# bluenote-1577/sylph

Measured on AMD Instinct MI355X. Metric: read Gbp/s sketched + genome-comparisons/s profiled, 1 Gbp vs GTDB-R220, higher is better.
Workload: dtype u64

## Files before the change

sylph_amd/csrc/common.h:

```cpp
#pragma once
#include <hip/hip_runtime.h>

#include <atomic>
#include <cstdarg>
#include <cstdint>
#include <cstdio>
#include <cstdlib>
#include <cstring>
#include <ctime>
#include <map>
#include <mutex>
#include <string>
#include <vector>

#include "../../include/sylph_hip.h"

struct sylph_ctx;

namespace sylph {

void set_error(const char* fmt, ...);

struct HipError { hipError_t e; const char* what; const char* file; int line; };

// ... 49 lines not shown

void* pool_acquire(sylph_ctx* ctx, size_t bytes, size_t* cap_out);
void pool_release(sylph_ctx* ctx, void* p, size_t cap);

struct DevBuf {
    void* p = nullptr;
    size_t cap = 0;
    sylph_ctx* ctx = nullptr;
    DevBuf() = default;
    explicit DevBuf(sylph_ctx* c) : ctx(c) {}
    DevBuf(const DevBuf&) = delete;
    DevBuf& operator=(const DevBuf&) = delete;
    ~DevBuf() { release(); }
    void release() {
        if (p) {
            if (ctx) pool_release(ctx, p, cap);
            else (void)hipFree(p);
        }
        p = nullptr;
        cap = 0;
    }
    void alloc(size_t want) {
        if (ctx) p = pool_acquire(ctx, want, &cap);
        else { SY_HIP(hipMalloc(&p, want)); cap = want; }
    }
    void reserve(size_t bytes) {
        if (bytes <= cap) return;
        release();
        alloc(bytes + bytes / 4 + 256);
    }
    void grow_keep(size_t bytes, size_t keep, hipStream_t s) {
        if (bytes <= cap) return;
        void* old = p;
        const size_t old_cap = cap;
        p = nullptr;
        cap = 0;
        alloc(bytes * 2 + 256);
        if (keep && old) SY_HIP(hipMemcpyAsync(p, old, keep, hipMemcpyDeviceToDevice, s));
        if (old) {
            if (ctx) pool_release(ctx, old, old_cap);
            else { SY_HIP(hipStreamSynchronize(s)); (void)hipFree(old); }
        }
    }
    template <class T> T* as() const { return reinterpret_cast<T*>(p); }
};

struct KernelStat { double ms = 0; uint64_t launches = 0; };

}

#ifndef SYLPH_READS_TAIL_PCT
#define SYLPH_READS_TAIL_PCT 10
#endif
struct sylph_ctx {
    int device = 0;
    hipStream_t stream = nullptr;
    bool own_stream = false;
    std::mutex mu;
    int finish_mode = 0;
    uint32_t bucket_target = 128;
    uint32_t plain_records = 1;
    uint32_t shard_reduce = 0;
    uint32_t fail_next_peer_copy = 0;
    uint32_t fail_next_shard_probe = 0;
    uint32_t index_lambda = 0;
    uint64_t index_pass_max = 1ull << 30;
    struct SeedTurn { hipEvent_t gate = nullptr, done = nullptr; bool recorded = false; } turn;
    void seed_gate() { if (turn.gate) { (void)hipStreamWaitEvent(stream, turn.gate, 0); turn.gate = nullptr; } }
    void seed_done() { if (turn.done && !turn.recorded && hipEventRecord(turn.done, stream) == hipSuccess) turn.recorded = true; }
    std::string profile_only;
    uint32_t reads_tail_pct = SYLPH_READS_TAIL_PCT;
    int reads_hash = -1;
    uint32_t reads_slack = 0;
    uint32_t reads_wg_per_cu = 0;
    uint64_t push_chunk_bytes = 64ull << 20;
    int seeds_mode = 0;
    std::atomic<int> refs{1};
    bool profile = false;
    std::map<std::string, sylph::KernelStat> stats;
    struct Pending { std::string fam; hipEvent_t a, b; };
    std::vector<Pending> pending;
    std::vector<hipEvent_t> event_pool;
    std::vector<std::pair<size_t, void*>> pool_free;
    size_t pool_bytes = 0;
    sylph::DevBuf tmp_sort;
    sylph::DevBuf scratch[8];
    sylph::DevBuf counters;
    void* pinned = nullptr;
    void read_back(void* dst, const void* dev_src, size_t bytes);
    static constexpr size_t STAGE_BYTES = 32u << 20;
    void* stage[2] = {nullptr, nullptr};
    hipEvent_t stage_ev[2] = {nullptr, nullptr};
    hipStream_t copy_stream = nullptr;
    hipEvent_t copy_ev[2] = {nullptr, nullptr};
    void d2h(void* dst, const void* dev_src, size_t bytes);
    void h2d(void* dev_dst, const void* src, size_t bytes);
};

namespace sylph {

struct ScopedKernelTimer {
    sylph_ctx* ctx;
    hipEvent_t a = nullptr, b = nullptr;
    const char* fam;
    ScopedKernelTimer(sylph_ctx* c, const char* family);
    ~ScopedKernelTimer();
};
void profile_collect(sylph_ctx* ctx);
void ctx_unref(sylph_ctx* ctx);

struct HostPhase {
    sylph_ctx* ctx;
    const char* name;
// ... 36 lines not shown
```

sylph_amd/csrc/partition.h:

```cpp
#pragma once
#include "common.h"
#include "device_common.h"
#include "sketch_session.h"

namespace sylph {
namespace {

struct BucketMap { int sh; uint32_t mult; uint32_t B; int composite; uint32_t range_hs; uint32_t sub_mult[3]; uint32_t sub_width[3]; int rank_bits[3]; };

__device__ __forceinline__ uint32_t bucket_of_key(uint32_t key, const BucketMap m) { return min(__umulhi(key, m.mult), m.B - 1u); }
__device__ __forceinline__ uint64_t bucket_lo_hash(uint32_t b, uint32_t mult, int sh) { return ((((uint64_t)b << 32) + mult - 1u) / mult) << sh; }
__device__ __forceinline__ uint32_t sub_range_of(uint32_t res, uint32_t sub_mult, uint32_t cap) {
    return sub_mult ? min(__umulhi(res, sub_mult), cap - 1u) : min(res, cap - 1u);
}
__device__ __forceinline__ uint32_t take_place(uint16_t* fill, uint32_t bin) {
    const uint32_t old = atomicAdd(reinterpret_cast<uint32_t*>(fill) + (bin >> 1), (bin & 1u) ? 65536u : 1u);
    return (bin & 1u) ? (old >> 16) : (old & 0xFFFFu);
}

struct PartIn {
    const uint64_t* hash;
    const uint32_t* slot_key;
    const uint32_t* blk_count;
    uint32_t n_dense, n_blk, slot_cap, tile_entries;
    uint32_t blk_per_tile;
    int slotted, key_sh;
    uint32_t stage_pairs;
    int carry;
};
constexpr int PART_TPB = 256;
constexpr uint32_t BLK_PER_TILE = 16;
constexpr uint32_t MAX_COARSE = 4096;
constexpr uint32_t MAX_FINE = 4096;
#ifndef SYLPH_STAGE_PAIRS
#define SYLPH_STAGE_PAIRS 4096
#endif
constexpr uint32_t STAGE_PAIRS = SYLPH_STAGE_PAIRS;

__device__ __forceinline__ uint32_t xcd_tile(uint32_t n_tiles) {
    const uint32_t per_xcd = (n_tiles + 7) / 8;
    return (blockIdx.x & 7u) * per_xcd + (blockIdx.x >> 3);
}

template <class F>
__device__ __forceinline__ void for_tile_entries(const PartIn& in, uint32_t t, F&& f) {
    if (in.slotted == 1) {
        const uint32_t grp = threadIdx.x >> 5, l = threadIdx.x & 31;
        for (uint32_t bl = grp; bl < in.blk_per_tile; bl += PART_TPB / 32) {
            const uint32_t b = t * in.blk_per_tile + bl;
            if (b >= in.n_blk) break;
            const uint32_t cnt = min(in.blk_count[b], in.slot_cap), g0 = b * in.slot_cap;
            for (uint32_t i = l; i < cnt; i += 32) f(in.slot_key[g0 + i], g0 + i, 0ull);
        }
    } else if (in.slotted == 2) {
        const uint32_t grp = threadIdx.x >> 5, l = threadIdx.x & 31;
        for (uint32_t bl = grp; bl < in.blk_per_tile; bl += PART_TPB / 32) {
            const uint32_t b = t * in.blk_per_tile + bl;
            if (b >= in.n_blk) break;
            const uint32_t cnt = 2u * min(in.blk_count[b], in.slot_cap), g0 = 2u * b * in.slot_cap;
            for (uint32_t i = l; i < cnt; i += 32) {
                const uint64_t h = in.hash[g0 + i];
                if (h != INVALID_HASH) f((uint32_t)(h >> in.key_sh), g0 + i, h);
            }
        }
// ... 250 lines not shown
```

sylph_amd/csrc/replay_lds.hip:

```cpp
#include "common.h"
#include "device_common.h"
#include "sketch_session.h"
#include "partition.h"

namespace sylph {
namespace {

#ifndef SYLPH_REPLAY_TPB
#define SYLPH_REPLAY_TPB 128
#endif
constexpr int CAP_SMALL = 256, RTPB_SMALL = SYLPH_REPLAY_TPB;
constexpr int CAP_MID = 512, RTPB_MID = 256;
constexpr int CAP_LARGE = 1024, RTPB_LARGE = 256;
constexpr int IDX_BITS = 10;
constexpr uint32_t SEG_LIMIT = 96;


struct ReplayArgs {
    const OccRec* recs;
    const uint64_t* hash;
    const uint32_t* perm;
    const uint32_t* boff;
    const uint32_t* p_nv;
    int paired, dedup;
    uint32_t cutoff;
    BucketMap bm;
    uint64_t* tmp_k;
    uint32_t* tmp_c;
    uint32_t* n_distinct;
    uint32_t* removed_b;
    uint32_t* overflow;
    uint32_t* mid_list;
    uint32_t* large_list;
    uint32_t* ovf_list;
    int dbg_stage;
};

struct FinishTail {
    unsigned long long removed;
    uint32_t overflow;
    uint32_t n_seg;
    uint32_t n_ovf, n_mid, n_large;
    uint32_t verdict[2];
    uint32_t a10_words[2];
    uint32_t n_found;
};
static_assert(sizeof(FinishTail) == 48, "tail block");

__device__ __forceinline__ uint32_t marker_tag(uint64_t m) { return (uint32_t)((m * 0x9E3779B97F4A7C15ull) >> 49) | 1u; }

template <int CAP, int RTPB>
__device__ __forceinline__ void replay_bucket(const uint32_t b, const ReplayArgs& ra) {
    const OccRec* __restrict__ recs = ra.recs;
    const uint32_t* __restrict__ perm = ra.perm;
    const uint32_t* __restrict__ boff = ra.boff;
    uint64_t* __restrict__ tmp_k = ra.tmp_k;
    uint32_t* __restrict__ tmp_c = ra.tmp_c;
    uint32_t* __restrict__ n_distinct = ra.n_distinct;
    uint32_t* __restrict__ mid_list = ra.mid_list;
    const int paired = ra.paired, dbg_stage = ra.dbg_stage;
    const uint32_t cutoff = ra.cutoff;
    const BucketMap& bm = ra.bm;
    constexpr int ITEMS = CAP / RTPB;
    const bool filter = ra.dedup == DEDUP_FILTER;
    const int no_dedup = filter ? 0 : ra.dedup;
    __shared__ uint64_t s_hash[CAP], s_rid[CAP], s_m0[CAP], s_m1[CAP];
    __shared__ __attribute__((aligned(8))) uint16_t s_seg[CAP];
    __shared__ uint8_t s_fl[CAP];
    __shared__ __attribute__((aligned(8))) uint16_t s_ab[2 * (CAP + 2)];
    uint16_t* const s_a = s_ab;
    uint16_t* const s_b = s_ab + (CAP + 2);
    __shared__ uint32_t s_wave[RTPB / 64];
    const uint32_t tid = threadIdx.x;
    const uint32_t nv = *ra.p_nv;
    const uint32_t first = boff[b], last = boff[b + 1];
    const uint32_t n = last - first;
    if (last > nv || first > last) { if (tid == 0) atomicAdd(ra.overflow, 1u); return; }
    if (n == 0) return;
    if (n > CAP) {
        if (tid == 0) {
            uint32_t* list = (CAP < CAP_MID && n <= (uint32_t)CAP_MID) ? mid_list : (CAP < CAP_LARGE && n <= (uint32_t)CAP_LARGE) ? ra.large_list : ra.ovf_list;
            list[1 + atomicAdd(&list[0], 1u)] = b;
        }
        return;
    }
    uint64_t* s_key = s_m0;
    const bool composite = bm.composite != 0;
    const uint64_t lo_hash = composite ? bucket_lo_hash(b, bm.mult, bm.sh) : 0ull;
    OccRec r[ITEMS];
    uint32_t pidx[ITEMS], rank[ITEMS];
    constexpr bool SEG_DIRECT = CAP == CAP_SMALL;
    uint32_t seg0[ITEMS];
#pragma unroll
    for (int q = 0; q < ITEMS; q++) seg0[q] = 0;
    uint32_t* const s_pidx = reinterpret_cast<uint32_t*>(s_rid);
    const int levels = (int)((n + RTPB - 1) / RTPB);
#pragma unroll
    for (int q = 0; q < ITEMS; q++) pidx[q] = perm[first + min(tid + q * RTPB, n - 1u)];
#pragma unroll
    for (int q = 0; q < ITEMS; q++) r[q] = recs[pidx[q]];
#pragma unroll
    for (int q = 0; q < ITEMS; q++) {
        rank[q] = 0;
        if (tid + q * RTPB >= n) pidx[q] = 0xFFFFFFFFu;
    }
    if (composite) {
        uint32_t* const s_cnt = reinterpret_cast<uint32_t*>(s_m1);
        const uint32_t sub_mult = bm.sub_mult[CAP == CAP_SMALL ? 0 : CAP == CAP_MID ? 1 : 2];
        uint32_t sub[ITEMS];
        constexpr int CFG = CAP == CAP_SMALL ? 0 : CAP == CAP_MID ? 1 : 2;
        const int rank_bits = bm.rank_bits[CFG];
        constexpr bool TWO_LEVEL = CAP != CAP_SMALL;
        unsigned long long* const s_min = reinterpret_cast<unsigned long long*>(s_hash);
        unsigned long long* const s_max = reinterpret_cast<unsigned long long*>(s_rid);
        for (uint32_t t = tid; t <= (uint32_t)CAP; t += RTPB) s_cnt[t] = 0;
        for (uint32_t t = tid; t < (uint32_t)CAP / 2; t += RTPB) reinterpret_cast<uint32_t*>(s_seg)[t] = 0;
        if constexpr (TWO_LEVEL)
            for (uint32_t t = tid; t < (uint32_t)CAP; t += RTPB) { s_min[t] = ~0ull; s_max[t] = 0ull; }
        __syncthreads();
#pragma unroll
        for (int q = 0; q < ITEMS; q++) {
            const uint32_t i = tid + q * RTPB;
            sub[q] = 0;
            if (i < n) {
                sub[q] = sub_range_of((uint32_t)((r[q].hash - lo_hash) >> bm.sh), sub_mult, CAP);
// ... 376 lines not shown
    {
        uint32_t rc = base_c;
        for (uint32_t t = 0; t < items; t++) {
            const uint32_t j = j0 + t;
            if (j >= n) break;
            s_b[j] = (uint16_t)rc;
            if (cbits & (1u << t)) rc++;
        }
        if (j0 < n && j0 + items >= n) s_b[n] = (uint16_t)rc;
    }
    __syncthreads();
    }
    if constexpr (HASHED) {
        uint16_t* const s_headpos = s_a;
        {
            uint32_t rh = base_h;
            for (uint32_t t = 0; t < items; t++) {
                const uint32_t j = j0 + t;
                if (j >= n) break;
                if (headbits & (1u << t)) s_headpos[rh++] = (uint16_t)j;
            }
            if (tid == 0) s_headpos[total_heads] = (uint16_t)n;
        }
        __syncthreads();
        uint32_t rh = base_h;
        for (uint32_t t = 0; t < items; t++) {
            const uint32_t j = j0 + t;
            if (j >= n) break;
            if (headbits & (1u << t)) {
                const uint32_t e = s_headpos[rh + 1];
                tmp_k[first + rh] = s_hash[j];
                tmp_c[first + rh] = (uint32_t)s_b[e] - (uint32_t)s_b[j];
                rh++;
            }
        }
    } else {
        uint32_t rh = base_h;
        const uint32_t out0 = first;
        for (uint32_t t = 0; t < items; t++) {
            const uint32_t j = j0 + t;
            if (j >= n) break;
            if (headbits & (1u << t)) {
                uint32_t e = j + 1;
                while (e < n && s_seg[e] == j) e++;
                tmp_k[out0 + rh] = s_hash[j];
                tmp_c[out0 + rh] = (uint32_t)s_b[e] - (uint32_t)s_b[j];
                rh++;
            }
        }
    }
    if (tid == 0) { n_distinct[b] = total_heads; ra.removed_b[b] = total_removed; }
}

template <int CAP, int RTPB>
__global__ __launch_bounds__(RTPB) void bucket_replay_kernel(ReplayArgs ra) {
    replay_bucket<CAP, RTPB>(blockIdx.x, ra);
}

template <int CAP, int RTPB>
__device__ __forceinline__ void count_bucket(const uint32_t b, const ReplayArgs& ra) {
    const uint64_t* __restrict__ hash = ra.hash;
    const uint32_t* __restrict__ perm = ra.perm;
    const uint32_t* __restrict__ boff = ra.boff;
    uint64_t* __restrict__ tmp_k = ra.tmp_k;
    uint32_t* __restrict__ tmp_c = ra.tmp_c;
    const BucketMap& bm = ra.bm;
    constexpr int ITEMS = CAP / RTPB;
    __shared__ uint64_t s_key[CAP], s_sorted[CAP];
    __shared__ uint32_t s_cnt[CAP + 1], s_mult[CAP];
    __shared__ __attribute__((aligned(8))) uint16_t s_fill[CAP];
    __shared__ uint32_t s_wave[RTPB / 64];
    const uint32_t tid = threadIdx.x;
    const uint32_t nv = *ra.p_nv;
    const uint32_t first = boff[b], last = boff[b + 1];
    const uint32_t n = last - first;
    if (last > nv || first > last) { if (tid == 0) atomicAdd(ra.overflow, 1u); return; }
    if (n == 0) return;
    if (n > (uint32_t)CAP) {
        if (tid == 0) {
            uint32_t* list = (CAP < CAP_LARGE && n <= (uint32_t)CAP_LARGE) ? ra.large_list : ra.ovf_list;
            list[1 + atomicAdd(&list[0], 1u)] = b;
        }
        return;
    }
    const uint64_t lo_hash = bucket_lo_hash(b, bm.mult, bm.sh);
    const uint32_t sub_mult = bm.sub_mult[CAP == CAP_SMALL ? 0 : CAP == CAP_MID ? 1 : 2];
    uint64_t h[ITEMS];
    uint32_t sub[ITEMS], place[ITEMS];
#pragma unroll
    for (int q = 0; q < ITEMS; q++) {
        const uint32_t i = tid + q * RTPB;
        h[q] = i < n ? (perm ? hash[perm[first + i]] : hash[first + i]) : 0ull;
    }
    for (uint32_t t = tid; t <= (uint32_t)CAP; t += RTPB) s_cnt[t] = 0;
    for (uint32_t t = tid; t < (uint32_t)CAP; t += RTPB) s_fill[t] = 0;
    __syncthreads();
#pragma unroll
    for (int q = 0; q < ITEMS; q++) {
        const uint32_t i = tid + q * RTPB;
        sub[q] = 0;
        if (i < n) {
            sub[q] = sub_range_of((uint32_t)((h[q] - lo_hash) >> bm.sh), sub_mult, CAP);
            atomicAdd(&s_cnt[sub[q]], 1u);
        }
    }
    __syncthreads();
    scan_counters<CAP, RTPB>(s_cnt, s_cnt, s_wave);
    __syncthreads();
#pragma unroll
// ... 7 lines not shown
    }
    __syncthreads();
#pragma unroll
    for (int q = 0; q < ITEMS; q++) {
        const uint32_t i = tid + q * RTPB;
        if (i < n) {
            const uint32_t lo = s_cnt[sub[q]], hi = s_cnt[sub[q] + 1];
            uint32_t less = 0, eq = 0, eq_before = 0;
            for (uint32_t p = lo; p < hi; p++) {
                const uint64_t kp = s_key[p];
                less += kp < h[q] ? 1u : 0u;
                const uint32_t same = kp == h[q] ? 1u : 0u;
                eq += same;
                eq_before += (same && p < place[q]) ? 1u : 0u;
            }
            const uint32_t r = lo + less + eq_before;
            s_sorted[r] = h[q];
            s_mult[r] = eq_before == 0 ? eq : 0u;
        }
    }
    __syncthreads();
    const uint32_t items = (n + RTPB - 1) / RTPB, j0 = tid * items;
    uint32_t heads = 0;
    for (uint32_t t = 0; t < items; t++) {
        const uint32_t j = j0 + t;
        if (j >= n) break;
        heads += s_mult[j] ? 1u : 0u;
    }
    uint32_t total_heads = 0;
    uint32_t rh = block_excl_sum<RTPB>(heads, s_wave, &total_heads);
    for (uint32_t t = 0; t < items; t++) {
        const uint32_t j = j0 + t;
        if (j >= n) break;
        const uint32_t m = s_mult[j];
        if (m) { tmp_k[first + rh] = s_sorted[j]; tmp_c[first + rh] = m; rh++; }
    }
    if (tid == 0) { ra.n_distinct[b] = total_heads; ra.removed_b[b] = 0; }
}
template <int CAP, int RTPB>
__global__ __launch_bounds__(RTPB) void bucket_count_kernel(ReplayArgs ra) {
    count_bucket<CAP, RTPB>(blockIdx.x, ra);
}
template <int CAP, int RTPB>
__global__ __launch_bounds__(RTPB) void bucket_count_list_kernel(ReplayArgs ra, const uint32_t* __restrict__ my_list) {
    const uint32_t n_listed = my_list[0];
    for (uint32_t i = blockIdx.x; i < n_listed; i += gridDim.x) {
        count_bucket<CAP, RTPB>(my_list[1 + i], ra);
        __syncthreads();
    }
}
template <int CAP, int RTPB>
__global__ __launch_bounds__(RTPB) void bucket_replay_list_kernel(ReplayArgs ra, const uint32_t* __restrict__ my_list) {
    const uint32_t n_listed = my_list[0];
    for (uint32_t i = blockIdx.x; i < n_listed; i += gridDim.x) {
        replay_bucket<CAP, RTPB>(my_list[1 + i], ra);
        __syncthreads();
    }
}

constexpr uint32_t SCAN_CHUNK = 1024;
__global__ __launch_bounds__(SCAN_CHUNK) void table_scan_kernel(const uint32_t* __restrict__ n_distinct, const uint32_t* __restrict__ removed_b,
                                                                uint32_t B, uint32_t ipt, uint32_t* __restrict__ d_loc,
                                                                uint32_t* __restrict__ chunk_rows, unsigned long long* __restrict__ chunk_removed) {
    __shared__ uint32_t s_wave[SCAN_CHUNK / 64];
    __shared__ unsigned long long s_rem[SCAN_CHUNK / 64];
    const uint32_t b0 = (blockIdx.x * SCAN_CHUNK + threadIdx.x) * ipt, lane = threadIdx.x & 63, wave = threadIdx.x >> 6;
    uint32_t v = 0;
    unsigned long long rem = 0;
    for (uint32_t i = 0; i < ipt && b0 + i < B; i++) { v += n_distinct[b0 + i]; rem += removed_b[b0 + i]; }
    uint32_t x = v;
#pragma unroll
    for (int d = 1; d < 64; d <<= 1) {
        const uint32_t y = __shfl_up(x, d);
        if (lane >= (uint32_t)d) x += y;
    }
#pragma unroll
    for (int d = 32; d > 0; d >>= 1) rem += __shfl_xor(rem, d);
    if (lane == 63) s_wave[wave] = x;
    if (lane == 0) s_rem[wave] = rem;
    __syncthreads();
    uint32_t base = 0, tot = 0;
    for (uint32_t w = 0; w < SCAN_CHUNK / 64; w++) { const uint32_t t = s_wave[w]; if (w < wave) base += t; tot += t; }
    uint32_t run = base + x - v;
    for (uint32_t i = 0; i < ipt && b0 + i < B; i++) { d_loc[b0 + i] = run; run += n_distinct[b0 + i]; }
    if (threadIdx.x == 0) {
        unsigned long long r = 0;
        for (uint32_t w = 0; w < SCAN_CHUNK / 64; w++) r += s_rem[w];
        chunk_rows[blockIdx.x] = tot;
        chunk_removed[blockIdx.x] = r;
    }
}
__global__ __launch_bounds__(256) void table_compact_kernel(const uint64_t* __restrict__ tmp_k, const uint32_t* __restrict__ tmp_c,
                                                            const uint32_t* __restrict__ boff, const uint32_t* __restrict__ d_loc,
                                                            const uint32_t* __restrict__ chunk_rows, const unsigned long long* __restrict__ chunk_removed,
                                                            const uint32_t* __restrict__ n_distinct, uint32_t B, uint32_t ipt,
                                                            uint64_t* __restrict__ out_k, uint32_t* __restrict__ out_c,
                                                            const uint32_t* __restrict__ ovf_list, const uint32_t* __restrict__ mid_list,
                                                            const uint32_t* __restrict__ large_list, int skip_if_listed,
                                                            FinishTail* __restrict__ tail, const uint32_t* __restrict__ verdict,
                                                            const uint32_t* __restrict__ a10_words, const uint32_t* __restrict__ p_nv) {
    __shared__ uint32_t s_base[257];
    __shared__ uint32_t s_wave[4];
    __shared__ unsigned long long s_rem[4];
    const uint32_t chunk = SCAN_CHUNK * ipt, n_chunks = (B + chunk - 1) / chunk;
    {
        const uint32_t v = threadIdx.x < n_chunks ? chunk_rows[threadIdx.x] : 0u;
        uint32_t tot = 0;
        const uint32_t ex = block_excl_sum<256>(v, s_wave, &tot);
// ... 35 lines not shown
        uint32_t run = 0;
        for (uint32_t t = 0; t < 1024; t++) { const uint32_t v = s_part[t]; s_part[t] = run; run += v; }
        sub_off[m] = run;
    }
    __syncthreads();
    uint32_t run = s_part[tid];
    for (uint32_t i = tid * per; i < min(m, (tid + 1) * per); i++) {
        const uint32_t b = ovf_list[1 + i];
        sub_off[i] = run;
        run += boff[b + 1] - boff[b];
    }
}

__global__ __launch_bounds__(256) void ovf_indices_kernel(const uint32_t* __restrict__ ovf_list, const uint32_t* __restrict__ sub_off,
                                                          const uint32_t* __restrict__ boff, const uint32_t* __restrict__ perm,
                                                          uint32_t* __restrict__ sub_idx) {
    const uint32_t b = ovf_list[1 + blockIdx.x], first = boff[b], n = boff[b + 1] - first, o = sub_off[blockIdx.x];
    for (uint32_t j = threadIdx.x; j < n; j += blockDim.x) sub_idx[o + j] = perm[first + j];
}
__global__ __launch_bounds__(256) void ovf_gather_kernel(const uint32_t* __restrict__ sorted_idx, uint32_t n, const OccRec* __restrict__ recs,
                                                         uint64_t* __restrict__ sub_hash, OccRec* __restrict__ sub_recs) {
    const uint32_t j = blockIdx.x * blockDim.x + threadIdx.x;
    if (j >= n) return;
    const OccRec r = recs[sorted_idx[j]];
    sub_hash[j] = r.hash;
    sub_recs[j] = r;
}

__global__ __launch_bounds__(256) void ovf_patch_kernel(const uint32_t* __restrict__ ovf_list, BucketMap bm,
                                                        const uint64_t* __restrict__ sub_k, const uint32_t* __restrict__ sub_c,
                                                        uint32_t n_sub_out, const uint32_t* __restrict__ boff,
                                                        uint64_t* __restrict__ tmp_k, uint32_t* __restrict__ tmp_c,
                                                        uint32_t* __restrict__ n_distinct) {
    const uint32_t b = ovf_list[1 + blockIdx.x];
    auto lower = [&](uint64_t key) {
        uint32_t lo = 0, hi = n_sub_out;
        while (lo < hi) {
            const uint32_t mid = lo + ((hi - lo) >> 1);
            if (sub_k[mid] < key) lo = mid + 1; else hi = mid;
        }
        return lo;
    };
    __shared__ uint32_t s_lo, s_hi;
    if (threadIdx.x == 0) {
        s_lo = lower(bucket_lo_hash(b, bm.mult, bm.sh));
        s_hi = (b + 1 < bm.B) ? lower(bucket_lo_hash(b + 1, bm.mult, bm.sh)) : n_sub_out;
    }
    __syncthreads();
    const uint32_t lo = s_lo, n = s_hi - s_lo, d = boff[b];
    for (uint32_t i = threadIdx.x; i < n; i += blockDim.x) { tmp_k[d + i] = sub_k[lo + i]; tmp_c[d + i] = sub_c[lo + i]; }
    if (threadIdx.x == 0) n_distinct[b] = n;
}

uint32_t grid_of(uint64_t n, uint32_t tpb = 256) { return (uint32_t)((n + tpb - 1) / tpb); }

}

bool finish_bucketed(sylph_sketch* sk) {
    sylph_ctx* ctx = sk->ctx;
    const bool slotted = sk->pend.live;
    const bool deferred = slotted && sk->pend.deferred;
    const uint32_t n_cap = slotted ? sk->pend.n : (uint32_t)sk->n_occ;
    const uint32_t n_all = deferred ? std::max<uint32_t>(1, sk->pend.n_expect) : n_cap;
    sk->n_out = 0;
    sk->dup_removed = 0;
    if (n_cap == 0) return true;
    if (sk->c < 2) return false;
    const uint64_t thr = UINT64_MAX / (uint64_t)sk->c;
    const uint32_t TARGET = ctx->bucket_target;
    const uint32_t B = (uint32_t)std::min<uint64_t>(std::max<uint64_t>(1, n_all / TARGET), 1u << 24);
    BucketMap bm;
    bm.sh = key_shift(sk->c);
    const uint64_t hs_max = thr >> bm.sh;
    bm.mult = (uint32_t)std::min<uint64_t>(0xFFFFFFFFull, ((uint64_t)B << 32) / (hs_max + 1));
    bm.B = B;
    const uint64_t range_hs = (0x100000000ull + bm.mult - 1) / std::max<uint32_t>(1, bm.mult) + 1;
    bm.composite = bm.mult >= 1 && bit_length(range_hs) + bm.sh <= 64 - IDX_BITS;
    bm.range_hs = (uint32_t)std::min<uint64_t>(range_hs, 0xFFFFFFFFull);
    {
        const uint32_t caps[3] = {(uint32_t)CAP_SMALL, (uint32_t)CAP_MID, (uint32_t)CAP_LARGE};
        for (int i = 0; i < 3; i++) bm.sub_mult[i] = range_hs > caps[i] ? (uint32_t)(((uint64_t)caps[i] << 32) / range_hs) : 0u;
        const uint64_t max_index = slotted ? (uint64_t)sk->pend.n_blk * sk->pend.slot_cap : (uint64_t)n_all;
        const int index_bits = bit_length(max_index | 1);
        for (int i = 0; i < 3; i++) {
            bm.sub_width[i] = bm.sub_mult[i] ? (uint32_t)(range_hs / caps[i]) : 1u;
            uint64_t span_hs = 1;
            if (bm.sub_mult[i]) {
                const uint64_t top = std::min<uint64_t>(range_hs, (((uint64_t)caps[i] << 32) + bm.sub_mult[i] - 1) / bm.sub_mult[i]);
                span_hs = top - (uint64_t)(caps[i] - 1) * bm.sub_width[i] + 1;
            }
            bm.rank_bits[i] = (bm.composite && bit_length(span_hs) + bm.sh + index_bits <= 64) ? index_bits : 0;
        }
    }
    const PartGeom geom = part_geometry(B);
    if (!slotted && sk->n_plain && !(sk->n_plain == sk->n_occ && bm.composite)) materialise_plain_records(sk);
    bool plain = !slotted && sk->n_plain != 0;
    static const uint32_t tile_blocks = [] { const char* e = getenv("SYLPH_HIP_PART_TILE_BLOCKS"); return e ? (uint32_t)std::max(1, std::min(32, atoi(e))) : BLK_PER_TILE; }();
    static const uint32_t stage_pairs = [] { const char* e = getenv("SYLPH_HIP_PART_STAGE_PAIRS"); return e ? (uint32_t)std::max(256, std::min(8192, atoi(e))) : 2048u; }();
    PartIn in{};
    in.slotted = slotted ? 1 : 0;
    in.key_sh = bm.sh;
    uint32_t n_tiles;
    const OccRec* recs;
    if (slotted) {
        in.slot_key = sk->slot_key.as<uint32_t>();
        in.n_blk = sk->pend.n_blk;
        in.slot_cap = sk->pend.slot_cap;
        in.blk_count = sk->slot_meta.as<uint32_t>() + (sk->pend.n_blk + 1);
        in.blk_per_tile = tile_blocks;
        in.stage_pairs = stage_pairs;
        n_tiles = (in.n_blk + tile_blocks - 1) / tile_blocks;
        recs = sk->slot_rec.as<OccRec>();
    } else {
        in.hash = sk->hash.as<uint64_t>();
        in.n_dense = n_all;
        in.tile_entries = (uint32_t)std::max<uint64_t>(4096, ((uint64_t)n_all + 65535) / 65536);
        n_tiles = (uint32_t)(((uint64_t)n_all + in.tile_entries - 1) / in.tile_entries);
        recs = sk->recs.as<OccRec>();
    }
    DevBuf &b_hist = ctx->scratch[0], &b_pairs = ctx->scratch[1], &b_perm = ctx->scratch[2], &b_tmpk = ctx->scratch[3],
           &b_tmpc = ctx->scratch[4], &b_small = ctx->scratch[5], &b_bk = ctx->scratch[6];
    b_hist.reserve(part_hist_words(geom, n_tiles) * 4);
    b_pairs.reserve((size_t)n_cap * 8);
    if (!plain) b_perm.reserve((size_t)n_cap * 4);
    DevBuf& b_sorted = ctx->scratch[7];
    if (plain) b_sorted.reserve((size_t)n_cap * 8);
    uint64_t* sorted_hash = plain ? b_sorted.as<uint64_t>() : nullptr;
    in.carry = plain ? 1 : 0;
    b_tmpk.reserve((size_t)n_cap * 8);
    b_tmpc.reserve((size_t)n_cap * 4);
    b_small.reserve(64);
    b_bk.reserve((size_t)(B + 2) * 4 * 7 + 264 * 4 + 264 * 8 + 16);
    uint32_t* hist = b_hist.as<uint32_t>();
    uint2* pairs = b_pairs.as<uint2>();
    uint32_t* boff = b_bk.as<uint32_t>();
    uint32_t* large_list = boff + (B + 2);
    uint32_t* ovf_list = large_list + (B + 2);
    uint32_t* n_distinct = ovf_list + (B + 2);
    uint32_t* removed_b = n_distinct + (B + 2);
    uint32_t* d_off = removed_b + (B + 2);
    uint32_t* mid_list = d_off + (B + 2);
    uint32_t* chunk_rows = mid_list + (B + 2) + ((B & 1u) ? 1 : 0);
    unsigned long long* chunk_removed = reinterpret_cast<unsigned long long*>(chunk_rows + 264);
    FinishTail* d_tail = b_small.as<FinishTail>();
    const uint32_t* d_nv = boff + B;
    const uint32_t n_zero = (B + 2) * 2;
    const int dbg = getenv("SYLPH_REPLAY_STAGE") ? atoi(getenv("SYLPH_REPLAY_STAGE")) : 0;
    const uint32_t cutoff = sk->paired ? 0u : 4u;
    sk->out_k.reserve((size_t)n_cap * 8);
    sk->out_c.reserve((size_t)n_cap * 4);
    ReplayArgs ra{};
    if (plain) ra.hash = sorted_hash;
    else { ra.recs = recs; ra.perm = b_perm.as<uint32_t>(); }
    ra.boff = boff; ra.p_nv = d_nv;
    ra.paired = sk->paired; ra.dedup = sk->dedup_mode(); ra.cutoff = cutoff; ra.bm = bm;
    ra.tmp_k = b_tmpk.as<uint64_t>(); ra.tmp_c = b_tmpc.as<uint32_t>(); ra.n_distinct = n_distinct; ra.removed_b = removed_b;
    ra.overflow = &d_tail->overflow;
    ra.mid_list = mid_list; ra.large_list = large_list; ra.ovf_list = ovf_list; ra.dbg_stage = dbg;
    {
        HostPhase ph(ctx, "finish(bucket): partition + LDS replay + compact");
        {
            ScopedKernelTimer t(ctx, "sort");
            launch_partition(ctx, in, bm, geom, n_tiles, n_all, hist, pairs, boff, b_perm.as<uint32_t>(), sorted_hash, n_distinct, n_zero,
                             b_small.as<uint32_t>(), large_list, ovf_list, mid_list);
        }
        {
            ScopedKernelTimer t(ctx, "replay");
            if (plain) hipLaunchKernelGGL((bucket_count_kernel<CAP_SMALL, RTPB_SMALL>), dim3(B), dim3(RTPB_SMALL), 0, ctx->stream, ra);
            else hipLaunchKernelGGL((bucket_replay_kernel<CAP_SMALL, RTPB_SMALL>), dim3(B), dim3(RTPB_SMALL), 0, ctx->stream, ra);
        }
    }
    auto close_table = [&](int skip_if_listed) {
        const uint32_t ipt = (B + (1u << 18) - 1) >> 18;
        ScopedKernelTimer t(ctx, "replay");
        hipLaunchKernelGGL(table_scan_kernel, dim3((B + SCAN_CHUNK * ipt - 1) / (SCAN_CHUNK * ipt)), dim3(SCAN_CHUNK), 0, ctx->stream, n_distinct,
                           removed_b, B, ipt, d_off, chunk_rows, chunk_removed);
        hipLaunchKernelGGL(table_compact_kernel, dim3(std::min<uint32_t>((B + 3) / 4, 1u << 15)), dim3(256), 0, ctx->stream,
                           b_tmpk.as<uint64_t>(), b_tmpc.as<uint32_t>(), boff, d_off, chunk_rows, chunk_removed, n_distinct, B, ipt,
                           sk->out_k.as<uint64_t>(), sk->out_c.as<uint32_t>(), ovf_list, mid_list, large_list, skip_if_listed,
                           d_tail, deferred ? sk->slot_meta.as<uint32_t>() + (size_t)(sk->pend.n_blk + 1) * 4 : (const uint32_t*)nullptr,
                           sk->a10_state == 1 ? sk->a10_tail.as<uint32_t>() : (const uint32_t*)nullptr, d_nv);
        SY_HIP(hipGetLastError());
    };
    FinishTail host{};
    auto read_tail = [&] {
        SY_HIP(hipMemcpyAsync(ctx->pinned, d_tail, sizeof host, hipMemcpyDeviceToHost, ctx->stream));
        SY_HIP(hipStreamSynchronize(ctx->stream));
        memcpy(&host, ctx->pinned, sizeof host);
        if (!ctx->pending.empty()) profile_collect(ctx);
    };
    close_table(1);
    read_tail();
    if (deferred) {
        if (host.verdict[0] || host.verdict[1]) {
            redo_deferred_batch(sk);
            a10_mark(sk);
            return finish_bucketed(sk);
        }
        sk->pend.deferred = false;
        sk->pend.n = host.n_found;
    }
    if (!a10_verdict(sk, host.a10_words)) return finish_bucketed(sk);
    if (host.overflow) return false;
    if (plain && host.n_ovf) {
        materialise_plain_records(sk);
        return finish_bucketed(sk);
    }
    if (host.n_mid || host.n_large) {
        HostPhase ph(ctx, "finish(bucket): medium / large configurations");
        {
            ScopedKernelTimer t(ctx, "replay");
            if (plain) {
                if (host.n_large)
                    hipLaunchKernelGGL((bucket_count_list_kernel<CAP_LARGE, RTPB_LARGE>), dim3(std::min<uint32_t>(host.n_large, 1536u)),
                                       dim3(RTPB_LARGE), 0, ctx->stream, ra, large_list);
            } else {
                if (host.n_mid)
                    hipLaunchKernelGGL((bucket_replay_list_kernel<CAP_MID, RTPB_MID>), dim3(std::min<uint32_t>(host.n_mid, 1280u)),
                                       dim3(RTPB_MID), 0, ctx->stream, ra, mid_list);
                if (host.n_large)
                    hipLaunchKernelGGL((bucket_replay_list_kernel<CAP_LARGE, RTPB_LARGE>), dim3(std::min<uint32_t>(host.n_large, 512u)),
                                       dim3(RTPB_LARGE), 0, ctx->stream, ra, large_list);
            }
        }
        close_table(0);
        read_tail();
        if (host.overflow) return false;
    }
    unsigned long long removed_extra = 0;
    if (host.n_ovf) {
        if (ctx->finish_mode == 2 || host.n_ovf > 4096) return false;
        HostPhase ph(ctx, "finish(bucket): overflowing buckets through the device-wide path");
        const uint32_t m = host.n_ovf;
        DevBuf b_so(ctx), b_si(ctx), b_sh(ctx), b_sr(ctx), sub_k(ctx), sub_c(ctx);
        b_so.reserve(((size_t)m + 1) * 4);
        hipLaunchKernelGGL(ovf_offsets_kernel, dim3(1), dim3(1024), 0, ctx->stream, ovf_list, boff, b_so.as<uint32_t>());
        uint32_t n_sub = 0;
        ctx->read_back(&n_sub, b_so.as<uint32_t>() + m, 4);
        b_si.reserve((size_t)n_sub * 8);
        b_sh.reserve((size_t)n_sub * 8);
        b_sr.reserve((size_t)n_sub * sizeof(OccRec));
        uint32_t* sub_idx = b_si.as<uint32_t>();
        uint32_t* sub_sorted = sub_idx + n_sub;
        hipLaunchKernelGGL(ovf_indices_kernel, dim3(m), dim3(256), 0, ctx->stream, ovf_list, b_so.as<uint32_t>(), boff,
                           b_perm.as<uint32_t>(), sub_idx);
        sort_keys_u32(ctx, sub_idx, sub_sorted, n_sub, 0, 32);
        {
            ScopedKernelTimer t(ctx, "replay_overflow");
            hipLaunchKernelGGL(ovf_gather_kernel, dim3(grid_of(n_sub)), dim3(256), 0, ctx->stream, sub_sorted, n_sub, recs,
                               b_sh.as<uint64_t>(), b_sr.as<OccRec>());
        }
        uint64_t n_sub_out = 0, removed_sub = 0;
        generic_replay(ctx, b_sh.as<uint64_t>(), b_sr.as<OccRec>(), n_sub, sk->paired, sk->dedup_mode(), sub_k, sub_c, n_sub_out, removed_sub);
        removed_extra = removed_sub;
        {
            ScopedKernelTimer t(ctx, "replay");
// ... 13 lines not shown
```

Before: 1110.

## Add a single-pass lane path for small buckets in replay and lower bucket target

Adds a specialized replay body for buckets holding at most 128 records. Each thread owns one record, ranks it by a direct count within its sub-range, and deduplicates without the general multi-item sort machinery. Specialised instances are templated on paired/dedup mode. The default bucket target drops from 128 to 96 so more buckets fit the lane path. The change also adds a reciprocal-based bucket low-key computation, moves shared memory into a struct shared by both bodies, and adds profiling counters; the extra template instances and the SGPR cap may raise register pressure.

New measurement: 1134, median of 6. +2.2%, better.

```diff
diff --git a/sylph_amd/csrc/common.h b/sylph_amd/csrc/common.h
--- a/sylph_amd/csrc/common.h
+++ b/sylph_amd/csrc/common.h
@@ -125,13 +125,16 @@
 #ifndef SYLPH_READS_TAIL_PCT
 #define SYLPH_READS_TAIL_PCT 10
 #endif
+#ifndef SYLPH_BUCKET_TARGET
+#define SYLPH_BUCKET_TARGET 96
+#endif
 struct sylph_ctx {
     int device = 0;
     hipStream_t stream = nullptr;
     bool own_stream = false;
     std::mutex mu;
     int finish_mode = 0;
-    uint32_t bucket_target = 128;
+    uint32_t bucket_target = SYLPH_BUCKET_TARGET;
     uint32_t plain_records = 1;
     uint32_t shard_reduce = 0;
     uint32_t fail_next_peer_copy = 0;
diff --git a/sylph_amd/csrc/partition.h b/sylph_amd/csrc/partition.h
--- a/sylph_amd/csrc/partition.h
+++ b/sylph_amd/csrc/partition.h
@@ -6,10 +6,16 @@
 namespace sylph {
 namespace {
 
-struct BucketMap { int sh; uint32_t mult; uint32_t B; int composite; uint32_t range_hs; uint32_t sub_mult[3]; uint32_t sub_width[3]; int rank_bits[3]; };
+struct BucketMap { int sh; uint32_t mult; uint32_t B; int composite; uint32_t range_hs; uint32_t sub_mult[4]; uint32_t sub_width[4]; int rank_bits[4]; uint64_t inv_mult; };
 
 __device__ __forceinline__ uint32_t bucket_of_key(uint32_t key, const BucketMap m) { return min(__umulhi(key, m.mult), m.B - 1u); }
 __device__ __forceinline__ uint64_t bucket_lo_hash(uint32_t b, uint32_t mult, int sh) { return ((((uint64_t)b << 32) + mult - 1u) / mult) << sh; }
+__device__ __forceinline__ uint64_t bucket_lo_key(uint32_t b, uint32_t mult, uint64_t inv) {
+    uint64_t q = (uint64_t)b * (uint32_t)(inv >> 32) + (((uint64_t)b * (uint32_t)inv) >> 32);
+    uint64_t r = ((uint64_t)b << 32) - q * mult;
+    if (r >= mult) { q++; r -= mult; }
+    return q + (r ? 1u : 0u);
+}
 __device__ __forceinline__ uint32_t sub_range_of(uint32_t res, uint32_t sub_mult, uint32_t cap) {
     return sub_mult ? min(__umulhi(res, sub_mult), cap - 1u) : min(res, cap - 1u);
 }
diff --git a/sylph_amd/csrc/replay_lds.hip b/sylph_amd/csrc/replay_lds.hip
--- a/sylph_amd/csrc/replay_lds.hip
+++ b/sylph_amd/csrc/replay_lds.hip
@@ -14,6 +14,8 @@
 constexpr int CAP_LARGE = 1024, RTPB_LARGE = 256;
 constexpr int IDX_BITS = 10;
 constexpr uint32_t SEG_LIMIT = 96;
+constexpr uint32_t SINGLE_CUTOFF = 4;
+constexpr int LANE_CAP = 128, LANE_CFG = 3;
 
 
 struct ReplayArgs {
@@ -47,10 +49,19 @@
 };
 static_assert(sizeof(FinishTail) == 48, "tail block");
 
+template <int CAP, int RTPB>
+struct ReplayLds {
+    uint64_t hash[CAP], rid[CAP], m0[CAP], m1[CAP];
+    __attribute__((aligned(8))) uint16_t seg[CAP];
+    uint8_t fl[CAP];
+    __attribute__((aligned(8))) uint16_t ab[2 * (CAP + 2)];
+    uint32_t wave[RTPB / 64];
+};
+
 __device__ __forceinline__ uint32_t marker_tag(uint64_t m) { return (uint32_t)((m * 0x9E3779B97F4A7C15ull) >> 49) | 1u; }
 
 template <int CAP, int RTPB>
-__device__ __forceinline__ void replay_bucket(const uint32_t b, const ReplayArgs& ra) {
+__device__ __forceinline__ void replay_bucket(const uint32_t b, const ReplayArgs& ra, ReplayLds<CAP, RTPB>& lds) {
     const OccRec* __restrict__ recs = ra.recs;
     const uint32_t* __restrict__ perm = ra.perm;
     const uint32_t* __restrict__ boff = ra.boff;
@@ -64,13 +75,13 @@
     constexpr int ITEMS = CAP / RTPB;
     const bool filter = ra.dedup == DEDUP_FILTER;
     const int no_dedup = filter ? 0 : ra.dedup;
-    __shared__ uint64_t s_hash[CAP], s_rid[CAP], s_m0[CAP], s_m1[CAP];
-    __shared__ __attribute__((aligned(8))) uint16_t s_seg[CAP];
-    __shared__ uint8_t s_fl[CAP];
-    __shared__ __attribute__((aligned(8))) uint16_t s_ab[2 * (CAP + 2)];
+    uint64_t* const s_hash = lds.hash, * const s_rid = lds.rid, * const s_m0 = lds.m0, * const s_m1 = lds.m1;
+    uint16_t* const s_seg = lds.seg;
+    uint8_t* const s_fl = lds.fl;
+    uint16_t* const s_ab = lds.ab;
     uint16_t* const s_a = s_ab;
     uint16_t* const s_b = s_ab + (CAP + 2);
-    __shared__ uint32_t s_wave[RTPB / 64];
+    uint32_t* const s_wave = lds.wave;
     const uint32_t tid = threadIdx.x;
     const uint32_t nv = *ra.p_nv;
     const uint32_t first = boff[b], last = boff[b + 1];
@@ -553,9 +564,181 @@
     if (tid == 0) { n_distinct[b] = total_heads; ra.removed_b[b] = total_removed; }
 }
 
-template <int CAP, int RTPB>
-__global__ __launch_bounds__(RTPB) void bucket_replay_kernel(ReplayArgs ra) {
-    replay_bucket<CAP, RTPB>(blockIdx.x, ra);
+template <bool PAIRED, int DEDUP>
+__device__ __forceinline__ void replay_bucket_lane(const uint32_t b, const uint32_t first, const uint32_t n, const ReplayArgs& ra,
+                                                   ReplayLds<CAP_SMALL, LANE_CAP>& lds) {
+    const OccRec* __restrict__ recs = ra.recs;
+    const uint32_t* __restrict__ perm = ra.perm;
+    uint64_t* __restrict__ tmp_k = ra.tmp_k;
+    uint32_t* __restrict__ tmp_c = ra.tmp_c;
+    const BucketMap& bm = ra.bm;
+    constexpr bool filter = DEDUP == DEDUP_FILTER, no_dedup = DEDUP == DEDUP_NONE;
+    uint64_t* const s_hash = lds.hash, * const s_rid = lds.rid, * const s_m0 = lds.m0, * const s_m1 = lds.m1;
+    uint16_t* const s_seg = lds.seg;
+    uint16_t* const s_a = lds.ab;
+    uint16_t* const s_b = lds.ab + (CAP_SMALL + 2);
+    uint32_t* const s_wave = lds.wave;
+    const uint32_t tid = threadIdx.x;
+    const bool live = tid < n;
+    const uint32_t pidx = perm[first + min(tid, n - 1u)];
+    const OccRec r = recs[pidx];
+    const uint64_t lo_hash = bucket_lo_key(b, bm.mult, bm.inv_mult) << bm.sh;
+    const int rank_bits = bm.rank_bits[LANE_CFG];
+    uint64_t* const s_key = s_m0;
+    uint32_t* const s_cnt = reinterpret_cast<uint32_t*>(s_m1);
+    uint16_t* const s_fill = s_seg;
+    s_cnt[tid] = 0;
+    if (tid == 0) s_cnt[LANE_CAP] = 0;
+    if (tid < LANE_CAP / 2) reinterpret_cast<uint32_t*>(s_seg)[tid] = 0;
+    __syncthreads();
+    uint32_t sub = 0;
+    if (live) {
+        sub = sub_range_of((uint32_t)((r.hash - lo_hash) >> bm.sh), bm.sub_mult[LANE_CFG], LANE_CAP);
+        atomicAdd(&s_cnt[sub], 1u);
+    }
+    __syncthreads();
+    {
+        const bool deep = scan_counters<LANE_CAP, LANE_CAP>(s_cnt, s_cnt, s_wave) >= SEG_LIMIT;
+        if constexpr (!no_dedup) {
+            if (__syncthreads_or(deep)) {
+                if (tid == 0) ra.mid_list[1 + atomicAdd(&ra.mid_list[0], 1u)] = b;
+                return;
+            }
+        } else
+            __syncthreads();
+    }
+    uint64_t rkey = 0;
+    if (live) {
+        const uint32_t place = s_cnt[sub] + take_place(s_fill, sub);
+        const uint64_t res = (r.hash - lo_hash) - ((uint64_t)(sub * bm.sub_width[LANE_CFG]) << bm.sh);
+        rkey = (res << rank_bits) | pidx;
+        s_key[place] = rkey;
+    }
+    __syncthreads();
+    uint32_t rank = 0, seg0 = 0;
+    if (live) {
+        const uint32_t lo = s_cnt[sub], hi = s_cnt[sub + 1];
+        const uint64_t hkey = rkey & ~((1ull << rank_bits) - 1ull);
+        uint32_t smaller = 0, below = 0;
+        for (uint32_t p = lo; p < hi; p++) {
+            const uint64_t kp = s_key[p];
+            smaller += kp < rkey ? 1u : 0u;
+            below += kp < hkey ? 1u : 0u;
+        }
+        rank = lo + smaller;
+        seg0 = lo + below;
+    }
+    __syncthreads();
+    if (live) {
+        s_hash[rank] = r.hash; s_rid[rank] = r.rid; s_m0[rank] = r.m0; s_m1[rank] = r.m1;
+        s_seg[rank] = (uint16_t)seg0;
+    }
+    __syncthreads();
+    const uint32_t j = tid;
+    const uint32_t seg = live ? (uint32_t)s_seg[j] : 0u;
+    const bool head = live && seg == j;
+    const uint64_t rid = live ? s_rid[j] : 0ull;
+    uint32_t* const s_tag = reinterpret_cast<uint32_t*>(lds.ab);
+    bool skip = false;
+    if (live) {
+        if constexpr (PAIRED) {
+            const uint64_t rec = rid & RID_MASK;
+            if (rec & 1) {
+                for (uint32_t q = j; q > seg;) {
+                    q--;
+                    const uint64_t rq = s_rid[q] & RID_MASK;
+                    if ((rq >> 1) != (rec >> 1)) break;
+                    if ((rq & 1) == 0) { skip = true; break; }
+                }
+            }
+        }
+        if constexpr (!filter && !no_dedup)
+            s_tag[j] = (!skip && (rid & RID_MARKER_BIT)) ? (marker_tag(s_m0[j]) | (marker_tag(s_m1[j]) << 16)) : 0u;
+    }
+    if constexpr (!filter && !no_dedup) __syncthreads();
+    bool dup = false;
+    if (live && !skip && (rid & RID_MARKER_BIT)) {
+        if constexpr (filter) {
+            if (rid & RID_A10_BIT) {
+                const uint64_t rec0 = s_rid[seg] & RID_MASK;
+                bool walk_first = (rid & RID_MASK) == rec0;
+                if (walk_first) {
+                    const uint64_t rank_j = (rid >> RID_RANK_SHIFT) & RID_RANK_MAX;
+                    for (uint32_t q = seg; q < n && (uint32_t)s_seg[q] == seg && (s_rid[q] & RID_MASK) == rec0; q++)
+                        if (q != j && ((s_rid[q] >> RID_RANK_SHIFT) & RID_RANK_MAX) < rank_j) { walk_first = false; break; }
+                }
+                dup = !walk_first;
+            }
+        } else if constexpr (!no_dedup) {
+            const uint64_t a = s_m0[j], bb = s_m1[j];
+            bool hit = false;
+            const uint32_t ta = marker_tag(a) * 0x00010001u, tb = marker_tag(bb) * 0x00010001u;
+            for (uint32_t q = seg; q < j; q++) {
+                const uint32_t w = s_tag[q], za = w ^ ta, zb = w ^ tb;
+                if ((((za - 0x00010001u) & ~za) | ((zb - 0x00010001u) & ~zb)) & 0x80008000u) {
+                    const uint64_t x = s_m0[q], y = s_m1[q];
+                    if (w && (x == a || y == a || x == bb || y == bb)) { hit = true; break; }
+                }
+            }
+            dup = j != seg && (hit || a == bb);
+        }
+    }
+    const bool u = live && !skip && (no_dedup || !dup);
+    uint32_t base_h, total_heads, total_removed;
+    if constexpr (PAIRED) {
+        const bool removed = live && !skip && !u;
+        uint32_t tot = 0;
+        const uint32_t base = block_excl_sum<LANE_CAP>((u ? 1u : 0u) | (head ? 1u << 10 : 0u) | (removed ? 1u << 20 : 0u), s_wave, &tot);
+        base_h = (base >> 10) & 0x3FFu;
+        total_heads = (tot >> 10) & 0x3FFu;
+        total_removed = tot >> 20;
+        if (live) {
+            s_b[j] = (uint16_t)(base & 0x3FFu);
+            if (j + 1 == n) s_b[n] = (uint16_t)((base & 0x3FFu) + (u ? 1u : 0u));
+        }
+        __syncthreads();
+    } else {
+        uint32_t tot_uh = 0;
+        const uint32_t base_uh = block_excl_sum<LANE_CAP>((u ? 1u : 0u) | (head ? 1u << 16 : 0u), s_wave, &tot_uh);
+        base_h = base_uh >> 16;
+        total_heads = tot_uh >> 16;
+        if (live) s_a[j] = (uint16_t)(base_uh & 0xFFFFu);
+        __syncthreads();
+        bool c = false;
+        if (live && !skip) c = ((uint32_t)s_a[j] - (uint32_t)s_a[seg] >= SINGLE_CUTOFF) ? true : u;
+        const bool removed = live && !skip && !c;
+        uint32_t tot_cr = 0;
+        const uint32_t base_c = block_excl_sum<LANE_CAP>((c ? 1u : 0u) | (removed ? 1u << 16 : 0u), s_wave, &tot_cr) & 0xFFFFu;
+        total_removed = tot_cr >> 16;
+        if (live) {
+            s_b[j] = (uint16_t)base_c;
+            if (j + 1 == n) s_b[n] = (uint16_t)(base_c + (c ? 1u : 0u));
+        }
+        __syncthreads();
+    }
+    if (head) {
+        uint32_t e = j + 1;
+        while (e < n && s_seg[e] == j) e++;
+        tmp_k[first + base_h] = s_hash[j];
+        tmp_c[first + base_h] = (uint32_t)s_b[e] - (uint32_t)s_b[j];
+    }
+    if (tid == 0) { ra.n_distinct[b] = total_heads; ra.removed_b[b] = total_removed; }
+}
+
+constexpr int LANE_OFF = -1;
+constexpr int lane_mode(bool paired, int dedup) { return (paired ? 1 : 0) | (dedup << 1); }
+template <int CAP, int RTPB, int LANE = LANE_OFF>
+__global__ __launch_bounds__(RTPB) __attribute__((amdgpu_num_sgpr(100))) void bucket_replay_kernel(ReplayArgs ra) {
+    __shared__ ReplayLds<CAP, RTPB> lds;
+    if constexpr (LANE != LANE_OFF) {
+        static_assert(CAP == CAP_SMALL && RTPB == LANE_CAP, "the lane body shares the 256-slot configuration's workgroup");
+        const uint32_t first = ra.boff[blockIdx.x], last = ra.boff[blockIdx.x + 1];
+        if (first < last && last <= *ra.p_nv && last - first <= (uint32_t)LANE_CAP && ra.bm.composite && ra.bm.rank_bits[LANE_CFG]) {
+            replay_bucket_lane<(LANE & 1) != 0, (LANE >> 1)>(blockIdx.x, first, last - first, ra, lds);
+            return;
+        }
+    }
+    replay_bucket<CAP, RTPB>(blockIdx.x, ra, lds);
 }
 
 template <int CAP, int RTPB>
@@ -669,8 +852,9 @@
 template <int CAP, int RTPB>
 __global__ __launch_bounds__(RTPB) void bucket_replay_list_kernel(ReplayArgs ra, const uint32_t* __restrict__ my_list) {
     const uint32_t n_listed = my_list[0];
+    __shared__ ReplayLds<CAP, RTPB> lds;
     for (uint32_t i = blockIdx.x; i < n_listed; i += gridDim.x) {
-        replay_bucket<CAP, RTPB>(my_list[1 + i], ra);
+        replay_bucket<CAP, RTPB>(my_list[1 + i], ra, lds);
         __syncthreads();
     }
 }
@@ -812,6 +996,22 @@
     if (threadIdx.x == 0) n_distinct[b] = n;
 }
 
+void launch_replay(sylph_ctx* ctx, uint32_t B, const ReplayArgs& ra, bool paired, bool stage_cut) {
+    auto go = [&](auto kernel) { hipLaunchKernelGGL(kernel, dim3(B), dim3(RTPB_SMALL), 0, ctx->stream, ra); };
+    if constexpr (RTPB_SMALL == LANE_CAP) {
+        if (!stage_cut) {
+            if (paired && ra.dedup == DEDUP_EXACT) return go(bucket_replay_kernel<CAP_SMALL, RTPB_SMALL, lane_mode(true, DEDUP_EXACT)>);
+            if (paired && ra.dedup == DEDUP_FILTER) return go(bucket_replay_kernel<CAP_SMALL, RTPB_SMALL, lane_mode(true, DEDUP_FILTER)>);
+            if (!paired && ra.dedup == DEDUP_EXACT) return go(bucket_replay_kernel<CAP_SMALL, RTPB_SMALL, lane_mode(false, DEDUP_EXACT)>);
+        }
+    }
+    go(bucket_replay_kernel<CAP_SMALL, RTPB_SMALL>);
+}
+bool lane_road(const BucketMap& bm, uint32_t n, bool paired, int dedup, bool stage_cut) {
+    const bool instance = RTPB_SMALL == LANE_CAP && !stage_cut && (dedup == DEDUP_EXACT || (paired && dedup == DEDUP_FILTER));
+    return instance && n >= 1 && n <= (uint32_t)LANE_CAP && bm.composite && bm.rank_bits[LANE_CFG];
+}
+
 uint32_t grid_of(uint64_t n, uint32_t tpb = 256) { return (uint32_t)((n + tpb - 1) / tpb); }
 
 }
@@ -834,15 +1034,16 @@
     const uint64_t hs_max = thr >> bm.sh;
     bm.mult = (uint32_t)std::min<uint64_t>(0xFFFFFFFFull, ((uint64_t)B << 32) / (hs_max + 1));
     bm.B = B;
+    bm.inv_mult = bm.mult > 1 ? (uint64_t)(((unsigned __int128)1 << 64) / bm.mult) : ~0ull;
     const uint64_t range_hs = (0x100000000ull + bm.mult - 1) / std::max<uint32_t>(1, bm.mult) + 1;
     bm.composite = bm.mult >= 1 && bit_length(range_hs) + bm.sh <= 64 - IDX_BITS;
     bm.range_hs = (uint32_t)std::min<uint64_t>(range_hs, 0xFFFFFFFFull);
     {
-        const uint32_t caps[3] = {(uint32_t)CAP_SMALL, (uint32_t)CAP_MID, (uint32_t)CAP_LARGE};
-        for (int i = 0; i < 3; i++) bm.sub_mult[i] = range_hs > caps[i] ? (uint32_t)(((uint64_t)caps[i] << 32) / range_hs) : 0u;
+        const uint32_t caps[4] = {(uint32_t)CAP_SMALL, (uint32_t)CAP_MID, (uint32_t)CAP_LARGE, (uint32_t)LANE_CAP};
+        for (int i = 0; i < 4; i++) bm.sub_mult[i] = range_hs > caps[i] ? (uint32_t)(((uint64_t)caps[i] << 32) / range_hs) : 0u;
         const uint64_t max_index = slotted ? (uint64_t)sk->pend.n_blk * sk->pend.slot_cap : (uint64_t)n_all;
         const int index_bits = bit_length(max_index | 1);
-        for (int i = 0; i < 3; i++) {
+        for (int i = 0; i < 4; i++) {
             bm.sub_width[i] = bm.sub_mult[i] ? (uint32_t)(range_hs / caps[i]) : 1u;
             uint64_t span_hs = 1;
             if (bm.sub_mult[i]) {
@@ -906,7 +1107,7 @@
     const uint32_t* d_nv = boff + B;
     const uint32_t n_zero = (B + 2) * 2;
     const int dbg = getenv("SYLPH_REPLAY_STAGE") ? atoi(getenv("SYLPH_REPLAY_STAGE")) : 0;
-    const uint32_t cutoff = sk->paired ? 0u : 4u;
+    const uint32_t cutoff = sk->paired ? 0u : SINGLE_CUTOFF;
     sk->out_k.reserve((size_t)n_cap * 8);
     sk->out_c.reserve((size_t)n_cap * 4);
     ReplayArgs ra{};
@@ -927,7 +1128,7 @@
         {
             ScopedKernelTimer t(ctx, "replay");
             if (plain) hipLaunchKernelGGL((bucket_count_kernel<CAP_SMALL, RTPB_SMALL>), dim3(B), dim3(RTPB_SMALL), 0, ctx->stream, ra);
-            else hipLaunchKernelGGL((bucket_replay_kernel<CAP_SMALL, RTPB_SMALL>), dim3(B), dim3(RTPB_SMALL), 0, ctx->stream, ra);
+            else launch_replay(ctx, B, ra, sk->paired != 0, dbg != 0);
         }
     }
     auto close_table = [&](int skip_if_listed) {
@@ -962,6 +1163,18 @@
     }
     if (!a10_verdict(sk, host.a10_words)) return finish_bucketed(sk);
     if (host.overflow) return false;
+    if (ctx->profile && !plain && (ctx->profile_only.empty() || ctx->profile_only.find(",replay,") != std::string::npos)) {
+        std::vector<uint32_t> h_boff((size_t)B + 1);
+        ctx->d2h(h_boff.data(), boff, ((size_t)B + 1) * 4);
+        uint64_t n_lane = 0, n_general = 0;
+        for (uint32_t i = 0; i < B; i++) {
+            const uint32_t n_b = h_boff[i + 1] - h_boff[i];
+            if (lane_road(bm, n_b, sk->paired != 0, ra.dedup, dbg != 0)) n_lane++;
+            else if (n_b) n_general++;
+        }
+        ctx->stats["replay_lane"].launches += n_lane;
+        ctx->stats["replay_general"].launches += n_general;
+    }
     if (plain && host.n_ovf) {
         materialise_plain_records(sk);
         return finish_bucketed(sk);
```
